# kaisun24/CPU-Vision

Measured on AMD Instinct MI355X. Metric: Mpixels/sec on 3x3 conv2d, 4K fp32 frames, higher is better.
Workload: dtype f32

## Files before the change

cpu-vision_amd/csrc/conv3x3_c3.hip:

```cpp
#include <cstdlib>

#include "mv_common.h"
#include "mv_act.h"

namespace mv {

typedef float f32x16 __attribute__((ext_vector_type(16)));
typedef float f32x4 __attribute__((ext_vector_type(4)));


struct C3Args {
  const float* x;
  const float* w;
  const float* b;
  float* y;
  int cout, h, wdt;
  int mtiles;
  int th;
  int wc;
  int pitch;
  int tiles_x, tiles_y;
  int groups;
  int relu;
  int vec_rows;
  unsigned nblocks;
  float mean[3], stdv[3];
};

constexpr int kKS = 14;
constexpr int kK = 27;

__device__ constexpr int c3_row(int k) { return k / 3; }
__device__ constexpr int c3_dx(int k) { return k % 3; }

template <bool RELU>
__device__ inline float c3_act(float v) {
  if (RELU) v = relu_f32(v);
  return v;
}

template <bool RELU, bool FULL, bool FULLM, bool IN_U8>
__global__ __launch_bounds__(256, 2) void k_conv3x3_c3(const C3Args A) {
  extern __shared__ __attribute__((aligned(16))) float lds[];
  const int tid = threadIdx.x, lane = tid & (kWave - 1);
  const int wave = __builtin_amdgcn_readfirstlane(tid >> 6);
  const int l31 = lane & 31, hf = lane >> 5;
  const int cout = A.cout, h = A.h, w = A.wdt;
  const int th = A.th, wc = A.wc, pitch = A.pitch;
  const int tile_rows = th + 2;
  float* xin = lds;
  float* wfr = lds + 3 * tile_rows * pitch + 16;

  const unsigned wid = xcd_remap(blockIdx.x, A.nblocks);
  const int tx = wid % A.tiles_x;
  const unsigned t2 = wid / A.tiles_x;
  const int ty = t2 % A.tiles_y;
  const long long img = t2 / A.tiles_y;
  const int xb = tx * wc, yb = ty * th;
  const float* xp = A.x + (size_t)img * 3 * h * w;
  const uint8_t* xpu = reinterpret_cast<const uint8_t*>(A.x) + (size_t)img * 3 * h * w;
  const size_t plane = (size_t)h * w;
  auto norm = [&](unsigned byte, int ci) -> float {
    const float v = (float)byte * (float)(1.0 / 255.0);
    return (v - A.mean[ci]) / A.stdv[ci];
  };

  for (int q = wave; q < A.mtiles * kKS; q += 4) {
    const int s = q % kKS, m = q / kKS;
    const int co = 32 * m + l31, k = 2 * s + hf;
    float v = 0.f;
    if (co < cout && k < kK) v = A.w[(size_t)co * kK + k];
    if (co < cout && k == kK && A.b != nullptr) v = A.b[co];
    wfr[q * 64 + lane] = v;
  }
  {
    constexpr int kStage = 8;
    const int cols = wc + 2;
    const int rows_total = 3 * tile_rows;
    if (A.vec_rows) {
      const int nq = (wc + 8) >> 2;
      const int per_row = (nq + kWave - 1) / kWave;
      const int nitems = rows_total * per_row;
      for (int base = wave; base < nitems; base += 4 * kStage) {
        f32x4 v[kStage];
#pragma unroll
        for (int u = 0; u < kStage; ++u) {
          const int it = base + 4 * u;
          v[u] = (f32x4){0.f, 0.f, 0.f, 0.f};
          if (it < nitems) {
            const int r = it / per_row, q = (it - r * per_row) * kWave + lane;
            const int ci = r / tile_rows, rr = r - ci * tile_rows;
            const int gy = yb - 1 + rr, gx0 = xb - 4 + 4 * q;
            if (q < nq && gy >= 0 && gy < h && gx0 >= 0 && gx0 + 3 < w) {
              if constexpr (IN_U8) {
                const unsigned b4 = *reinterpret_cast<const unsigned*>(xpu + ((size_t)ci * h + gy) * w + gx0);
                v[u] = (f32x4){norm(b4 & 0xffu, ci), norm((b4 >> 8) & 0xffu, ci), norm((b4 >> 16) & 0xffu, ci), norm(b4 >> 24, ci)};
              } else {
                v[u] = *reinterpret_cast<const f32x4*>(xp + ((size_t)ci * h + gy) * w + gx0);
              }
            }
          }
        }
#pragma unroll
        for (int u = 0; u < kStage; ++u) {
          const int it = base + 4 * u;
          if (it < nitems) {
            const int r = it / per_row, q = (it - r * per_row) * kWave + lane;
            if (q < nq) {
              float* dst = xin + r * pitch + (4 * q - 3);
              const float e[4] = {v[u].x, v[u].y, v[u].z, v[u].w};
#pragma unroll
              for (int j = 0; j < 4; ++j) {
                const int c = 4 * q - 3 + j;
                if (c >= 0 && c < cols) dst[j] = e[j];
              }
            }
          }
        }
      }
    } else {
      const int per_row = (cols + kWave - 1) / kWave;
      const int nitems = rows_total * per_row;
      for (int base = wave; base < nitems; base += 4 * kStage) {
        float v[kStage];
#pragma unroll
        for (int u = 0; u < kStage; ++u) {
          const int it = base + 4 * u;
          v[u] = 0.f;
          if (it < nitems) {
            const int r = it / per_row, c = (it - r * per_row) * kWave + lane;
            const int ci = r / tile_rows, rr = r - ci * tile_rows;
            const int gy = yb - 1 + rr, gx = xb - 1 + c;
            if (c < cols && gy >= 0 && gy < h && gx >= 0 && gx < w) {
              if constexpr (IN_U8)
                v[u] = norm(xpu[((size_t)ci * h + gy) * w + gx], ci);
              else
                v[u] = xp[((size_t)ci * h + gy) * w + gx];
            }
          }
        }
#pragma unroll
        for (int u = 0; u < kStage; ++u) {
          const int it = base + 4 * u;
          if (it < nitems) {
            const int r = it / per_row, c = (it - r * per_row) * kWave + lane;
            if (c < cols) xin[r * pitch + c] = v[u];
          }
        }
      }
    }
  }
  __syncthreads();

  const int m = (A.mtiles == 2) ? (wave >> 1) : 0;
  const int gfirst = (A.mtiles == 2) ? (wave & 1) : wave;
  const int gstep = (A.mtiles == 2) ? 2 : 4;
  const int ng = (A.groups > gfirst) ? (A.groups - gfirst + gstep - 1) / gstep : 0;
  if (ng == 0) return;

  float afr[kKS];
#pragma unroll
  for (int s = 0; s < kKS; ++s) afr[s] = wfr[(m * kKS + s) * 64 + lane];

  int rowoff[9];
#pragma unroll
  for (int r = 0; r < 9; ++r) rowoff[r] = ((r / 3) * tile_rows + (r % 3)) * pitch;

  char* const simg = reinterpret_cast<char*>(A.y + (size_t)img * cout * plane);
  const unsigned chan_off = (unsigned)((size_t)(32 * m + 4 * hf) * plane * sizeof(float));

  auto geom = [&](int j, int& lbase, unsigned& voff, bool& ok) {
    const int g = gfirst + gstep * j;
    const unsigned f = 128u * (unsigned)g + 4u * (unsigned)l31;
    const unsigned ly = f / (unsigned)wc, lx = f - ly * (unsigned)wc;
    lbase = (int)(ly * (unsigned)pitch + lx);
    const int gy = yb + (int)ly, gx = xb + (int)lx;
    ok = FULL || (gy < h && gx < w && (int)ly < th);
    voff = chan_off + (unsigned)(((size_t)gy * w + gx) * sizeof(float));
  };
  auto load_row = [&](f32x4 (&dst)[2], int lbase, int r) {
    const float* p = xin + lbase + rowoff[r];
    dst[0] = *reinterpret_cast<const f32x4*>(p);
    dst[1] = *reinterpret_cast<const f32x4*>(p + 4);
  };
  auto elem = [](const f32x4 (&q)[2], int i) -> float {
    const f32x4& v = q[i >> 2];
    return (i & 3) == 0 ? v.x : (i & 3) == 1 ? v.y : (i & 3) == 2 ? v.z : v.w;
  };
  auto drain = [&](const f32x16 (&acc)[4], int i, unsigned voff, bool ok) {
    const int cu = (i & 3) + 8 * (i >> 2);
    f32x4 v = {c3_act<RELU>(acc[0][i]), c3_act<RELU>(acc[1][i]), c3_act<RELU>(acc[2][i]), c3_act<RELU>(acc[3][i])};
    f32x4* dst = reinterpret_cast<f32x4*>(simg + (size_t)cu * plane * sizeof(float) + voff);
    if ((FULL || ok) && (FULLM || 32 * m + cu + 4 * hf < cout)) *dst = v;
  };
  const f32x16 zero = {0.f, 0.f, 0.f, 0.f, 0.f, 0.f, 0.f, 0.f, 0.f, 0.f, 0.f, 0.f, 0.f, 0.f, 0.f, 0.f};

  f32x16 accA[4], accB[4];
  f32x4 row[9][2];
  f32x4 nrow[2][2];
  int lb_cur, lb_next;
  unsigned vo_cur, vo_prev = 0;
  bool ok_cur, ok_prev = false;
  geom(0, lb_cur, vo_cur, ok_cur);
  load_row(nrow[0], lb_cur, 0);
  load_row(nrow[1], lb_cur, 1);

#define MV_C3_GROUP(cur, prev, j, have_prev)                                                             \
  {                                                                                                      \
    unsigned vo_n = 0;                                                                                   \
    bool ok_n = false;                                                                                   \
    geom(min((j) + 1, ng - 1), lb_next, vo_n, ok_n);                                                      \
    row[0][0] = nrow[0][0], row[0][1] = nrow[0][1], row[1][0] = nrow[1][0], row[1][1] = nrow[1][1];       \
    _Pragma("unroll") for (int s = 0; s < kKS; ++s) {                                                    \
                    \
      constexpr_for_rows(s)                                                                              \
      _Pragma("unroll") for (int a = 0; a < 4; ++a) {                                                    \
        const int k0 = 2 * s, k1 = 2 * s + 1;                                                            \
        const float b0 = elem(row[c3_row(k0)], a + c3_dx(k0));                                           \
        const float b1 = (k1 < kK) ? elem(row[c3_row(k1 < kK ? k1 : 0)], a + c3_dx(k1)) : 1.0f;           \
        const float bsel = hf ? b1 : b0;                                                                 \
        cur[a] = __builtin_amdgcn_mfma_f32_32x32x2f32(afr[s], bsel, s == 0 ? zero : cur[a], 0, 0, 0);      \
        if (have_prev) {                                                                                 \
          const int slot = 4 * s + a;                                                                    \
          if (slot % 3 == 2 && slot / 3 < 16) drain(prev, slot / 3, vo_prev, ok_prev);                    \
        }                                                                                                \
      }                                                                                                  \
      if (s == 10) load_row(nrow[0], lb_next, 0);                                                        \
      if (s == 12) load_row(nrow[1], lb_next, 1);                                                        \
    }                                                                                                    \
    vo_prev = vo_cur, ok_prev = ok_cur;                                                                  \
    lb_cur = lb_next, vo_cur = vo_n, ok_cur = ok_n;                                                      \
  }
#define constexpr_for_rows(s)                                                                            \
  _Pragma("unroll") for (int r = 2; r < 9; ++r) {                                                        \
    if ((3 * r) / 2 - 1 == (s)) load_row(row[r], lb_cur, r);                                             \
  }

  MV_C3_GROUP(accA, accB, 0, false)
  int j = 1;
  for (; j + 1 < ng; j += 2) {
    MV_C3_GROUP(accB, accA, j, true)
    MV_C3_GROUP(accA, accB, j + 1, true)
  }
  if (j < ng) {
    MV_C3_GROUP(accB, accA, j, true)
#pragma unroll
    for (int i = 0; i < 16; ++i) drain(accB, i, vo_prev, ok_prev);
  } else {
#pragma unroll
    for (int i = 0; i < 16; ++i) drain(accA, i, vo_prev, ok_prev);
  }
#undef MV_C3_GROUP
#undef constexpr_for_rows
}

template <bool RELU, bool FULL, bool FULLM, bool IN_U8>
static int c3_launch_t(const C3Args& a, size_t lds_bytes, hipStream_t s) {
  auto k = k_conv3x3_c3<RELU, FULL, FULLM, IN_U8>;
  if (lds_bytes > 48 * 1024)
    (void)hipFuncSetAttribute(reinterpret_cast<const void*>(k), hipFuncAttributeMaxDynamicSharedMemorySize, (int)lds_bytes);
  hipLaunchKernelGGL(k, dim3(a.nblocks), dim3(256), lds_bytes, s, a);
  return check_launch("k_conv3x3_c3");
}

template <bool RELU, bool FULL, bool FULLM>
static int c3_launch(const C3Args& a, size_t lds_bytes, bool in_u8, hipStream_t s) {
  return in_u8 ? c3_launch_t<RELU, FULL, FULLM, true>(a, lds_bytes, s) : c3_launch_t<RELU, FULL, FULLM, false>(a, lds_bytes, s);
}

bool conv3x3_c3_supported(const float* x, const float* y, int cin, int cout, int h, int w) {
  const char* v = tune_env("MV_FORCE_GENERIC_CONV");
  if (v && *v && *v != '0') return false;
  if (cin != 3 || cout > 64 || cout < 1) return false;
  if (w % 4 != 0 || (uintptr_t)y % 16 != 0) return false;
  if ((size_t)cout * h * w * sizeof(float) >= (1ull << 32)) return false;
  (void)x;
  return true;
}

int launch_conv3x3_c3(const void* xv, bool in_u8, const float* mean3, const float* std3, const float* w, const float* b,
                      float* y, int64_t n, int h, int wdt, int cout, int relu, hipStream_t s) {
  C3Args a = {};
  const float* x = static_cast<const float*>(xv);
  a.x = x, a.w = w, a.b = b, a.y = y;
  for (int i = 0; i < 3; ++i) a.mean[i] = in_u8 ? mean3[i] : 0.f, a.stdv[i] = in_u8 ? std3[i] : 1.f;
  a.cout = cout, a.h = h, a.wdt = wdt, a.relu = relu;
  a.mtiles = (cout + 31) / 32;
  a.vec_rows = (wdt % 4 == 0) && ((uintptr_t)x % (in_u8 ? 4 : 16) == 0);
  const bool flat = wdt <= 256;
  a.wc = flat ? wdt : 256;
  a.pitch = ((a.wc + 2 + 3) & ~3) + 8;
  int th = 16;
  if (const char* e = tune_env("MV_C3_TH")) th = atoi(e) > 0 ? atoi(e) : th;
  auto bytes = [&](int rows) {
    return ((size_t)3 * (rows + 2) * a.pitch + 16 + (size_t)a.mtiles * kKS * 64) * sizeof(float);
  };
  while (th > 1 && bytes(th) > 150 * 1024) th >>= 1;
  if (!tune_env("MV_C3_TH"))
    while (th > 4 && (long long)n * ((wdt + a.wc - 1) / a.wc) * ((h + th - 1) / th) < 512) th >>= 1;
  if (th > h) th = h;
  a.th = th;
  a.tiles_x = (wdt + a.wc - 1) / a.wc;
  a.tiles_y = (h + th - 1) / th;
  a.groups = (th * a.wc + 127) / 128;
  const long long nb = (long long)n * a.tiles_x * a.tiles_y;
  if (nb > 0x7fffffffLL) return set_error(MV_ERR_UNSUPPORTED, "conv3x3: batch too large for one launch");
  a.nblocks = (unsigned)nb;
  const size_t lds_bytes = bytes(th);
  const bool full = (h % th == 0) && (wdt % a.wc == 0) && ((th * a.wc) % 128 == 0);
  const bool fullm = (cout % 32 == 0);
#define MV_C3_DISPATCH(R)                                                               \
  if (full && fullm) return c3_launch<R, true, true>(a, lds_bytes, in_u8, s);             \
  if (full) return c3_launch<R, true, false>(a, lds_bytes, in_u8, s);                     \
  if (fullm) return c3_launch<R, false, true>(a, lds_bytes, in_u8, s);                    \
  return c3_launch<R, false, false>(a, lds_bytes, in_u8, s);
  if (relu) {
    MV_C3_DISPATCH(true)
  }
  MV_C3_DISPATCH(false)
#undef MV_C3_DISPATCH
}

}
```

Before: 261,300.

## Use buffer stores with OOB clipping and incremental tile geometry in conv3x3 c3

Output stores now go through raw buffer stores built on a buffer resource descriptor. Out-of-range pixels and channels are sent to an offset past the record size, so the hardware drops them instead of the code branching on a predicate. Per-group geometry is advanced incrementally with add-and-wrap in place of a divide per group. The FULL/FULLM template variants are collapsed into a runtime channel check. This cuts template variants and address arithmetic, but adds s_nop and sched_barrier constraints around each store, which may limit instruction scheduling.

After: 262,400, median of 2. Within noise of the previous version (+0.4%).

```diff
diff --git a/cpu-vision_amd/csrc/conv3x3_c3.hip b/cpu-vision_amd/csrc/conv3x3_c3.hip
--- a/cpu-vision_amd/csrc/conv3x3_c3.hip
+++ b/cpu-vision_amd/csrc/conv3x3_c3.hip
@@ -1,4 +1,5 @@
 #include <cstdlib>
+#include <type_traits>
 
 #include "mv_common.h"
 #include "mv_act.h"
@@ -7,6 +8,7 @@
 
 typedef float f32x16 __attribute__((ext_vector_type(16)));
 typedef float f32x4 __attribute__((ext_vector_type(4)));
+typedef unsigned u32x4 __attribute__((ext_vector_type(4)));
 
 
 struct C3Args {
@@ -21,6 +23,7 @@
   int pitch;
   int tiles_x, tiles_y;
   int groups;
+  int step_rows, step_cols;
   int relu;
   int vec_rows;
   unsigned nblocks;
@@ -39,7 +42,7 @@
   return v;
 }
 
-template <bool RELU, bool FULL, bool FULLM, bool IN_U8>
+template <bool RELU, bool IN_U8>
 __global__ __launch_bounds__(256, 2) void k_conv3x3_c3(const C3Args A) {
   extern __shared__ __attribute__((aligned(16))) float lds[];
   const int tid = threadIdx.x, lane = tid & (kWave - 1);
@@ -152,34 +155,54 @@
   }
   __syncthreads();
 
-  const int m = (A.mtiles == 2) ? (wave >> 1) : 0;
-  const int gfirst = (A.mtiles == 2) ? (wave & 1) : wave;
-  const int gstep = (A.mtiles == 2) ? 2 : 4;
+  const unsigned plane_b = (unsigned)(plane * sizeof(float));
+  const unsigned nrec = (unsigned)cout * plane_b;
+  const __amdgpu_buffer_rsrc_t srd = __builtin_amdgcn_make_buffer_rsrc(A.y + (size_t)img * cout * plane, 0, (int)nrec, 0x00020000);
+  auto store4 = [&](auto check, const f32x4& v, int c, unsigned vo, unsigned vo_lo) {
+    const unsigned so = (unsigned)c * plane_b;
+    __builtin_amdgcn_sched_barrier(0);
+    if (!decltype(check)::value || c + 4 < cout) {
+      __builtin_amdgcn_raw_buffer_store_b128(__builtin_bit_cast(u32x4, v), srd, vo, so, 0);
+      asm volatile("s_nop 1");
+    } else if (c < cout) {
+      __builtin_amdgcn_raw_buffer_store_b128(__builtin_bit_cast(u32x4, v), srd, vo_lo, so, 0);
+      asm volatile("s_nop 1");
+    }
+    __builtin_amdgcn_sched_barrier(0);
+  };
+
+  const bool msplit = A.mtiles == 2;
+  const int m = msplit ? (wave >> 1) : 0;
+  const int gfirst = msplit ? (wave & 1) : wave, gstep = msplit ? 2 : 4;
   const int ng = (A.groups > gfirst) ? (A.groups - gfirst + gstep - 1) / gstep : 0;
   if (ng == 0) return;
 
-  float afr[kKS];
-#pragma unroll
-  for (int s = 0; s < kKS; ++s) afr[s] = wfr[(m * kKS + s) * 64 + lane];
+  struct Pos {
+    unsigned ly, lx, lb, pix;
+  };
+  const unsigned uwc = (unsigned)wc;
+  const unsigned rows_in = (unsigned)min(th, h - yb), cols_in = (unsigned)min(wc, w - xb);
+  const unsigned d_ly = (unsigned)A.step_rows, d_lx = (unsigned)A.step_cols;
+  const unsigned d_lb = d_ly * (unsigned)pitch + d_lx, d_pix = (d_ly * (unsigned)w + d_lx) * 4u;
+  const unsigned wrap_lb = (unsigned)(pitch - wc), wrap_pix = (unsigned)(w - wc) * 4u;
+  const unsigned lane_out = (unsigned)(4 * hf) * plane_b + ((unsigned)yb * (unsigned)w + (unsigned)xb) * 4u;
+  auto advance = [&](Pos& p) {
+    p.ly += d_ly, p.lx += d_lx, p.lb += d_lb, p.pix += d_pix;
+    if (p.lx >= uwc) p.lx -= uwc, p.ly += 1u, p.lb += wrap_lb, p.pix += wrap_pix;
+  };
+  auto out_off = [&](const Pos& p) -> unsigned { return (p.ly < rows_in && p.lx < cols_in) ? lane_out + p.pix : nrec; };
+  Pos pc;
+  {
+    const unsigned f = 128u * (unsigned)gfirst + 4u * (unsigned)l31;
+    pc.ly = f / uwc, pc.lx = f - pc.ly * uwc;
+    pc.lb = pc.ly * (unsigned)pitch + pc.lx, pc.pix = (pc.ly * (unsigned)w + pc.lx) * 4u;
+  }
 
   int rowoff[9];
 #pragma unroll
   for (int r = 0; r < 9; ++r) rowoff[r] = ((r / 3) * tile_rows + (r % 3)) * pitch;
-
-  char* const simg = reinterpret_cast<char*>(A.y + (size_t)img * cout * plane);
-  const unsigned chan_off = (unsigned)((size_t)(32 * m + 4 * hf) * plane * sizeof(float));
-
-  auto geom = [&](int j, int& lbase, unsigned& voff, bool& ok) {
-    const int g = gfirst + gstep * j;
-    const unsigned f = 128u * (unsigned)g + 4u * (unsigned)l31;
-    const unsigned ly = f / (unsigned)wc, lx = f - ly * (unsigned)wc;
-    lbase = (int)(ly * (unsigned)pitch + lx);
-    const int gy = yb + (int)ly, gx = xb + (int)lx;
-    ok = FULL || (gy < h && gx < w && (int)ly < th);
-    voff = chan_off + (unsigned)(((size_t)gy * w + gx) * sizeof(float));
-  };
-  auto load_row = [&](f32x4 (&dst)[2], int lbase, int r) {
-    const float* p = xin + lbase + rowoff[r];
+  auto load_row = [&](f32x4 (&dst)[2], unsigned lb, int r) {
+    const float* p = xin + lb + rowoff[r];
     dst[0] = *reinterpret_cast<const f32x4*>(p);
     dst[1] = *reinterpret_cast<const f32x4*>(p + 4);
   };
@@ -187,33 +210,33 @@
     const f32x4& v = q[i >> 2];
     return (i & 3) == 0 ? v.x : (i & 3) == 1 ? v.y : (i & 3) == 2 ? v.z : v.w;
   };
-  auto drain = [&](const f32x16 (&acc)[4], int i, unsigned voff, bool ok) {
-    const int cu = (i & 3) + 8 * (i >> 2);
-    f32x4 v = {c3_act<RELU>(acc[0][i]), c3_act<RELU>(acc[1][i]), c3_act<RELU>(acc[2][i]), c3_act<RELU>(acc[3][i])};
-    f32x4* dst = reinterpret_cast<f32x4*>(simg + (size_t)cu * plane * sizeof(float) + voff);
-    if ((FULL || ok) && (FULLM || 32 * m + cu + 4 * hf < cout)) *dst = v;
-  };
-  const f32x16 zero = {0.f, 0.f, 0.f, 0.f, 0.f, 0.f, 0.f, 0.f, 0.f, 0.f, 0.f, 0.f, 0.f, 0.f, 0.f, 0.f};
-
-  f32x16 accA[4], accB[4];
-  f32x4 row[9][2];
-  f32x4 nrow[2][2];
-  int lb_cur, lb_next;
-  unsigned vo_cur, vo_prev = 0;
-  bool ok_cur, ok_prev = false;
-  geom(0, lb_cur, vo_cur, ok_cur);
-  load_row(nrow[0], lb_cur, 0);
-  load_row(nrow[1], lb_cur, 1);
+
+  auto body = [&](auto check) {
+    f32x4 row[9][2];
+    float afr[kKS];
+#pragma unroll
+    for (int s = 0; s < kKS; ++s) afr[s] = wfr[(m * kKS + s) * 64 + lane];
+    auto drain = [&](const f32x16 (&acc)[4], int i, unsigned vo, unsigned vo_lo) {
+      const f32x4 v = {c3_act<RELU>(acc[0][i]), c3_act<RELU>(acc[1][i]), c3_act<RELU>(acc[2][i]), c3_act<RELU>(acc[3][i])};
+      store4(check, v, 32 * m + (i & 3) + 8 * (i >> 2), vo, vo_lo);
+    };
+    const f32x16 zero = {};
+    f32x16 accA[4], accB[4];
+    f32x4 nrow[2][2];
+    unsigned vo_prev = nrec, vlo_prev = nrec;
+    load_row(nrow[0], pc.lb, 0);
+    load_row(nrow[1], pc.lb, 1);
 
 #define MV_C3_GROUP(cur, prev, j, have_prev)                                                             \
   {                                                                                                      \
-    unsigned vo_n = 0;                                                                                   \
-    bool ok_n = false;                                                                                   \
-    geom(min((j) + 1, ng - 1), lb_next, vo_n, ok_n);                                                      \
+    Pos pn = pc;                                                                                         \
+    if ((j) + 1 < ng) advance(pn);                                                                       \
     row[0][0] = nrow[0][0], row[0][1] = nrow[0][1], row[1][0] = nrow[1][0], row[1][1] = nrow[1][1];       \
     _Pragma("unroll") for (int s = 0; s < kKS; ++s) {                                                    \
-                    \
-      constexpr_for_rows(s)                                                                              \
+         \
+      _Pragma("unroll") for (int r = 2; r < 9; ++r) {                                                    \
+        if ((3 * r) / 2 - 1 == s) load_row(row[r], pc.lb, r);                                            \
+      }                                                                                                  \
       _Pragma("unroll") for (int a = 0; a < 4; ++a) {                                                    \
         const int k0 = 2 * s, k1 = 2 * s + 1;                                                            \
         const float b0 = elem(row[c3_row(k0)], a + c3_dx(k0));                                           \
@@ -222,50 +245,45 @@
         cur[a] = __builtin_amdgcn_mfma_f32_32x32x2f32(afr[s], bsel, s == 0 ? zero : cur[a], 0, 0, 0);      \
         if (have_prev) {                                                                                 \
           const int slot = 4 * s + a;                                                                    \
-          if (slot % 3 == 2 && slot / 3 < 16) drain(prev, slot / 3, vo_prev, ok_prev);                    \
+          if (slot % 3 == 2 && slot / 3 < 16) drain(prev, slot / 3, vo_prev, vlo_prev);                   \
         }                                                                                                \
       }                                                                                                  \
-      if (s == 10) load_row(nrow[0], lb_next, 0);                                                        \
-      if (s == 12) load_row(nrow[1], lb_next, 1);                                                        \
+      if (s == 10) load_row(nrow[0], pn.lb, 0);                                                          \
+      if (s == 12) load_row(nrow[1], pn.lb, 1);                                                          \
     }                                                                                                    \
-    vo_prev = vo_cur, ok_prev = ok_cur;                                                                  \
-    lb_cur = lb_next, vo_cur = vo_n, ok_cur = ok_n;                                                      \
+    vo_prev = out_off(pc), vlo_prev = hf ? nrec : vo_prev;                                               \
+    pc = pn;                                                                                             \
   }
-#define constexpr_for_rows(s)                                                                            \
-  _Pragma("unroll") for (int r = 2; r < 9; ++r) {                                                        \
-    if ((3 * r) / 2 - 1 == (s)) load_row(row[r], lb_cur, r);                                             \
-  }
-
-  MV_C3_GROUP(accA, accB, 0, false)
-  int j = 1;
-  for (; j + 1 < ng; j += 2) {
-    MV_C3_GROUP(accB, accA, j, true)
-    MV_C3_GROUP(accA, accB, j + 1, true)
-  }
-  if (j < ng) {
-    MV_C3_GROUP(accB, accA, j, true)
-#pragma unroll
-    for (int i = 0; i < 16; ++i) drain(accB, i, vo_prev, ok_prev);
-  } else {
-#pragma unroll
-    for (int i = 0; i < 16; ++i) drain(accA, i, vo_prev, ok_prev);
-  }
+
+    MV_C3_GROUP(accA, accB, 0, false)
+    int j = 1;
+    for (; j + 1 < ng; j += 2) {
+      MV_C3_GROUP(accB, accA, j, true)
+      MV_C3_GROUP(accA, accB, j + 1, true)
+    }
+    if (j < ng) {
+      MV_C3_GROUP(accB, accA, j, true)
+#pragma unroll
+      for (int i = 0; i < 16; ++i) drain(accB, i, vo_prev, vlo_prev);
+    } else {
+#pragma unroll
+      for (int i = 0; i < 16; ++i) drain(accA, i, vo_prev, vlo_prev);
+    }
 #undef MV_C3_GROUP
-#undef constexpr_for_rows
-}
-
-template <bool RELU, bool FULL, bool FULLM, bool IN_U8>
+  };
+  if (cout == 32 * A.mtiles)
+    body(std::false_type{});
+  else
+    body(std::true_type{});
+}
+
+template <bool RELU, bool IN_U8>
 static int c3_launch_t(const C3Args& a, size_t lds_bytes, hipStream_t s) {
-  auto k = k_conv3x3_c3<RELU, FULL, FULLM, IN_U8>;
+  auto k = k_conv3x3_c3<RELU, IN_U8>;
   if (lds_bytes > 48 * 1024)
     (void)hipFuncSetAttribute(reinterpret_cast<const void*>(k), hipFuncAttributeMaxDynamicSharedMemorySize, (int)lds_bytes);
   hipLaunchKernelGGL(k, dim3(a.nblocks), dim3(256), lds_bytes, s, a);
   return check_launch("k_conv3x3_c3");
-}
-
-template <bool RELU, bool FULL, bool FULLM>
-static int c3_launch(const C3Args& a, size_t lds_bytes, bool in_u8, hipStream_t s) {
-  return in_u8 ? c3_launch_t<RELU, FULL, FULLM, true>(a, lds_bytes, s) : c3_launch_t<RELU, FULL, FULLM, false>(a, lds_bytes, s);
 }
 
 bool conv3x3_c3_supported(const float* x, const float* y, int cin, int cout, int h, int w) {
@@ -273,13 +291,15 @@
   if (v && *v && *v != '0') return false;
   if (cin != 3 || cout > 64 || cout < 1) return false;
   if (w % 4 != 0 || (uintptr_t)y % 16 != 0) return false;
-  if ((size_t)cout * h * w * sizeof(float) >= (1ull << 32)) return false;
+  if ((size_t)cout * h * w * sizeof(float) + 16 >= (1ull << 32)) return false;
   (void)x;
   return true;
 }
 
 int launch_conv3x3_c3(const void* xv, bool in_u8, const float* mean3, const float* std3, const float* w, const float* b,
                       float* y, int64_t n, int h, int wdt, int cout, int relu, hipStream_t s) {
+  if ((size_t)cout * h * wdt * sizeof(float) + 16 >= (1ull << 32))
+    return set_error(MV_ERR_UNSUPPORTED, "conv3x3: an image's output must stay below 2^32 - 16 bytes");
   C3Args a = {};
   const float* x = static_cast<const float*>(xv);
   a.x = x, a.w = w, a.b = b, a.y = y;
@@ -307,18 +327,10 @@
   if (nb > 0x7fffffffLL) return set_error(MV_ERR_UNSUPPORTED, "conv3x3: batch too large for one launch");
   a.nblocks = (unsigned)nb;
   const size_t lds_bytes = bytes(th);
-  const bool full = (h % th == 0) && (wdt % a.wc == 0) && ((th * a.wc) % 128 == 0);
-  const bool fullm = (cout % 32 == 0);
-#define MV_C3_DISPATCH(R)                                                               \
-  if (full && fullm) return c3_launch<R, true, true>(a, lds_bytes, in_u8, s);             \
-  if (full) return c3_launch<R, true, false>(a, lds_bytes, in_u8, s);                     \
-  if (fullm) return c3_launch<R, false, true>(a, lds_bytes, in_u8, s);                    \
-  return c3_launch<R, false, false>(a, lds_bytes, in_u8, s);
-  if (relu) {
-    MV_C3_DISPATCH(true)
-  }
-  MV_C3_DISPATCH(false)
-#undef MV_C3_DISPATCH
-}
-
-}
+  const int stride = a.mtiles == 2 ? 256 : 512;
+  a.step_rows = stride / a.wc, a.step_cols = stride % a.wc;
+  if (relu) return in_u8 ? c3_launch_t<true, true>(a, lds_bytes, s) : c3_launch_t<true, false>(a, lds_bytes, s);
+  return in_u8 ? c3_launch_t<false, true>(a, lds_bytes, s) : c3_launch_t<false, false>(a, lds_bytes, s);
+}
+
+}
```
